# volser/FluidFramework

Measured on AMD Instinct MI355X. Metric: sequenced merge-tree ops applied/sec (whole node) + achieved HBM GB/s, higher is better.
Workload: dtype int32; 1 GPU; config2: 4096 docs x 8 clients x 10k msgs, lag U[0,32], 60/40 ins/rem; docs_per_gpu=4096, msgs_per_doc=10000, clients=8, lag_max=32, parallelism=doc-sharded x1, residency=blk, big_min_ops=0

## Files before the change

fluidframework_amd/csrc/mt_core.h:

```cpp
#pragma once
#include <type_traits>
#include "wave.h"
#include "../../include/mtgpu.h"

#define MT_MAXH 16
#define MT_PSK 16
#define MT_PKEYS MT_MAX_PROP_KEYS
#ifndef MT_PATH_RESUME
#define MT_PATH_RESUME 1
#endif
#define MT_MAXN 8
#define MT_GRAN 256
#define MT_ZMAX 2
#define MT_NOREM 0x7FFFFFFF
#define MT_RFL 128
#ifndef MT_L_ROWS
#define MT_L_ROWS 256
#endif
#ifndef MT_L_BLKS
#define MT_L_BLKS 96
#endif
#ifndef MT_L_HEAP
#define MT_L_HEAP 96
#endif
#define MT_L_H 8
#ifndef MT_B_BLKS
#define MT_B_BLKS 104
#endif
#ifndef MT_B_SLACK
#define MT_B_SLACK 13
#endif
#define MT_B_BT 128
#ifndef MT_B_W
#define MT_B_W 64
#endif
#ifndef MT_B_HEAP
#define MT_B_HEAP 94
#endif
#ifndef MT_BW_BLKS
#define MT_BW_BLKS 248
#endif
#ifndef MT_BW_W
#define MT_BW_W 256
#endif
#ifndef MT_BW_HEAP
#define MT_BW_HEAP 254
#endif
#define MT_BW_BT 256
#ifndef MT_G_U
#define MT_G_U 768
#endif
#ifndef MT_G_HEAP
#define MT_G_HEAP 2046
#endif
#ifndef MT_G_WIN
#define MT_G_WIN 2048
#endif
#define MT_G_H 12
#ifndef MT_G_BCACHE
#define MT_G_BCACHE 0
#endif
#ifndef MT_G_BC
#define MT_G_BC (MT_G_BCACHE ? 512 : 1)
#endif
#ifndef MT_G_BCH
#define MT_G_BCH 1
#endif
#define MT_BC_EMPTY ((int)0x80000000)
#ifndef MT_G_NW
#define MT_G_NW 4
#endif
#define MT_G_STG 1024
#ifndef MT_G_MWMIN
#define MT_G_MWMIN 512
#endif
#ifndef MT_G_ALLCH
#define MT_G_ALLCH 0
#endif
enum { MT_MW_EXIT = 0, MT_MW_SCAN = 1, MT_MW_CHAIN = 2, MT_MW_PREFETCH = 3 };
enum { MT_BIGF_NO_BCACHE = 1, MT_BIGF_NO_PREFETCH = 2, MT_BIGF_NO_TABLE = 4, MT_BIGF_NO_BPC = 8 };
#ifndef MT_G_HT
#define MT_G_HT 4096
#endif
#ifndef MT_G_BPC
#define MT_G_BPC 1
#endif
#define MT_G_BPL 11
#define MT_G_BP (1 << MT_G_BPL)
#define MT_BP_EMPTY 0xFFFFFFFFu
#define MT_G_HTN (MT_G_HT * 3 / 4)
enum { MT_RES_HBM = 0, MT_RES_LDS = 1, MT_RES_BLK = 2, MT_RES_BIG = 3, MT_RES_BLKW = 4 };
#if defined(MT_PROFILE) || defined(MT_PROFILE2) || defined(MT_PROFILE3) || defined(MT_PROFILE4) || defined(MT_BPC_STATS) || defined(MT_EVCOUNT3) || defined(MT_EVCOUNT) || defined(MT_EVCOUNT2)
#define MT_KEEP_PROF 1
#else
#define MT_KEEP_PROF 0
#endif

#if defined(MT_PROFILE) && defined(__HIP_DEVICE_COMPILE__)
#define MT_PB(v) const unsigned long long v = __builtin_amdgcn_s_memtime()
#define MT_PE(i, v) prof[i] += __builtin_amdgcn_s_memtime() - (v)
#else
#define MT_PB(v)
#define MT_PE(i, v)
#endif
#if defined(MT_EVCOUNT)
#define MT_EV(i, v) prof[i] += (unsigned long long)(v)
#else
#define MT_EV(i, v)
#endif
#if defined(MT_EVCOUNT2)
#define MT_EV2(i, v) prof[i] += (unsigned long long)(v)
#else
#define MT_EV2(i, v)
#endif
#if defined(MT_PROFILE2) && defined(__HIP_DEVICE_COMPILE__)
#define MT_QB(v) const unsigned long long v = __builtin_amdgcn_s_memtime()
#define MT_QE(i, v) prof[i] += __builtin_amdgcn_s_memtime() - (v)
#define MT_QC(i) prof[i] += 1
#else
#define MT_QB(v)
#define MT_QE(i, v)
#define MT_QC(i)
#endif
#if defined(MT_PROFILE3) && defined(__HIP_DEVICE_COMPILE__)
#define MT_ZB(v) const unsigned long long v = __builtin_amdgcn_s_memtime()
#define MT_ZE(i, v) prof[i] += __builtin_amdgcn_s_memtime() - (v)
#define MT_ZC(i) prof[i] += 1
#else
#define MT_ZB(v)
#define MT_ZE(i, v)
#define MT_ZC(i)
#endif
#if defined(MT_BPC_STATS) && !defined(__HIP_DEVICE_COMPILE__)
#define MT_BS(i) prof[i] += 1
#else
#define MT_BS(i)
#endif
#if defined(MT_PROFILE4) && defined(__HIP_DEVICE_COMPILE__)
#define MT_UB(v) const unsigned long long v = __builtin_amdgcn_s_memtime()
#define MT_UE(i, v) prof[i] += __builtin_amdgcn_s_memtime() - (v)
#define MT_UC(i, x) prof[i] += (unsigned long long)(x)
#else
#define MT_UB(v)
#define MT_UE(i, v)
#define MT_UC(i, x)
#endif
enum { MT_PH_U = 0, MT_PH_SPLIT, MT_PH_INSERT, MT_PH_RANGE, MT_PH_ZAMBONI, MT_PH_OP, MT_PH_GEN, MT_PH_TEXT };

#define MT_M_CLIENT 0x0000FFFFu
#define MT_M_REMOVED 0x00010000u
#define MT_M_MARKER 0x00020000u
#define MT_M_INWIN 0x00040000u
#define MT_M_REG 0x00080000u
#define MT_M_NONL 0x00100000u
#define MT_M_HREF1 0x01000000u
#define MT_M_HREF 0xFF000000u

#ifndef MT_ROW64
#define MT_ROW64 0
#endif
struct __attribute__((aligned(16))) MtRow {
    int len;
    int seq;
    int rseq;
    uint32_t meta;
    int toff;
    int props;
    int parent;
    int tcap;
    unsigned long long ovl;
    uint32_t rcl;
    int mid;
#if MT_ROW64
    int pad[4];
#endif
};
struct __attribute__((aligned(16))) MtBlk {
    int c[8];
    int len;
    int parent;
    int n;
    int height;
    int scour;
    int pad[3];
};
struct __attribute__((aligned(16))) MtPSet {
    uint16_t key[MT_PSK];
    int32_t val[MT_PSK];
    int32_t n;
    int32_t pad[3];
};
struct MtHeapE { int seg; int maxSeq; };
struct MtOvx { int row; int rseq; int client; int pad; };
#define MT_OVX_CAP 512
#define MT_REG_CAP 64
struct MtReg { int client, name, n, flags, off, pad[3]; };
// ... 69 lines not shown
    int32_t seq, rseq;
    uint16_t rclient; int16_t prop;
    uint32_t poff, plen;
    uint32_t mid, pad1;
};
enum { MT_LD_START = 0, MT_LD_CONT = 1, MT_LD_REFLUSH = 2, MT_LD_REFLUSH_NEW = 3, MT_LD_UNSUPPORTED = 4 };
struct MtLoadStep { int seg, kind, cli, seq; };
struct MtLoad {
    const uint32_t* docs; const uint32_t* seg_off; const uint32_t* nhdr;
    const int32_t* ms; const int32_t* cs;
    const MtLoadSeg* segs; const uint16_t* payload;
    const uint32_t* plan_off; const MtLoadStep* plan;
};
#define MT_NONCOLLAB 0xFFFE
#define MT_NOBODY 0xFFFF

struct MtGen {
    unsigned long long seed;
    uint32_t ops, clients, lag_max, pct_insert, pct_remove, ins_len_max, rem_len_max, n_ann_sets, pct_rewrite;
    int enabled;
    const uint32_t* clients_per_run;
    uint32_t doc_id_base;
    uint32_t ins_len_min, seg_prop_sets, ins_at_end;
    uint64_t total_ops;
};

struct __attribute__((aligned(16))) MtQ16 { uint32_t x, y, z, w; };
struct __attribute__((aligned(16))) MtLdsPools {
    MtRow rows[MT_L_ROWS];
    MtBlk blk[MT_L_BLKS];
    MtHeapE heap[MT_L_HEAP + 2];
    int win[MT_L_ROWS];
    int uid[MT_L_ROWS];
    int udelta[MT_L_ROWS];
    uint8_t uanc[MT_L_ROWS * MT_L_H];
};

template <int NB, int NH, int NT, int NW> struct __attribute__((aligned(16))) MtLdsBlkT {
    static_assert(NB <= NT, "block ids index the corrections table");
    MtBlk blk[NB];
    MtHeapE heap[NH + 2];
    int win[NW];
    int bcorr[NT];
};
using MtLdsBlk = MtLdsBlkT<MT_B_BLKS, MT_B_HEAP, MT_B_BT, MT_B_W>;
using MtLdsBlkW = MtLdsBlkT<MT_BW_BLKS, MT_BW_HEAP, MT_BW_BT, MT_BW_W>;

struct __attribute__((aligned(16))) MtLdsBig {
    MtHeapE heap[MT_G_HEAP + 2];
    int win[MT_G_WIN];
    int uid[MT_G_U], udelta[MT_G_U];
    int uanc[MT_G_U * MT_G_H];
    uint16_t ulist[MT_G_U];
    MtBlk bc[MT_G_BC];
    int btag[MT_G_BC];
    int sid[MT_G_STG], sdel[MT_G_STG], spf[MT_G_STG];
    int htk[MT_G_HT], htv[MT_G_HT];
    uint16_t hlist[MT_G_HT];
    uint32_t bpc[MT_G_BP];
    struct Job {
        int op, r, c, r0, n, H, minSeq, heapN;
        MtRow* R; int* win; MtBlk* blk; int* uanc; uint16_t* text;
    } mw[2];
    int posted;
};

struct MtScratch {
    int pathB[MT_MAXH + 2], pathJ[MT_MAXH + 2];
    int pathOff[MT_MAXH + 2], pathLen[MT_MAXH + 2];
    int hold[64];
    int holdLen[64];
    uint8_t holdBlk[64];
    int rfree[MT_RFL];
    int corr[MT_MAXN];
};

struct __attribute__((aligned(16), may_alias)) MtQ16a { uint32_t x, y, z, w; };
#ifndef MT_NONL
#define MT_NONL 1
#endif
#ifndef MT_LEAF_ONCE
#define MT_LEAF_ONCE 1
#endif
#ifndef MT_GT_CH
#define MT_GT_CH 4
#endif
#ifndef MT_SCOUR_QUADS
#define MT_SCOUR_QUADS 1
#endif
MT_INLINE int pick16(const int* c, int j) {
    int v = c[0];
#pragma unroll
    for (int i = 1; i < 16; i++) v = (j == i) ? c[i] : v;
    return v;
}
MT_INLINE int pick8(const int* c, int j) {
    int v = c[0];
#pragma unroll
    for (int i = 1; i < 8; i++) v = (j == i) ? c[i] : v;
    return v;
}
MT_INLINE bool ovl_has(const MtOvx* ox, int n, unsigned long long ovl, int s, int rseq, int c) {
    if (c < 63) return ((ovl >> c) & 1ull) != 0;
    const bool more = (ovl >> 63) != 0;
    bool f = false;
    for (int i = 0; i < n; i++) {
        const MtOvx e = ox[i];
        f = f | (more & (e.row == s) & (e.client == c) & (e.rseq == rseq));
    }
    return f;
}
MT_INLINE bool vis_rc(int seq, uint32_t meta, int rseq, uint32_t rcl, unsigned long long ovl, int r, int c,
                      const MtOvx* ox, int nox, int s) {
    const int cl = (int)(meta & MT_M_CLIENT);
    const bool seen = (cl == c) | (seq <= r);
    const bool removed = (meta & MT_M_REMOVED) != 0;
    const bool gone = ((int)rcl == c) | (rseq <= r) | ovl_has(ox, nox, ovl, s, rseq, c);
    return seen & !(removed & gone);
}

struct BlkH { int len, parent, n, height, scour; };
struct ChildL { int len; bool tie; };
struct WinI { int id; int delta; int parent; bool live; bool recycle; };

enum { MT_WALK_SPLIT = 0, MT_WALK_INSERT = 1 };
enum { MT_W_OK = 0, MT_W_NOCHANGE = 1, MT_W_FAIL = 2 };
enum { MT_MAP_REMOVE = 0, MT_MAP_ANNOTATE = 1, MT_MAP_COLLECT = 2 };
enum { MT_PM_SET = 0, MT_PM_REWRITE = 1, MT_PM_INCR = 2, MT_PM_KEEP = 3, MT_PM_CONS = 4, MT_PM_INCR_SMIN = 5 };
MT_INLINE int mt_prop_mode(uint32_t fl) {
    if (!(fl & MT_OPF_COMBINE)) return (fl & MT_OPF_REWRITE) ? MT_PM_REWRITE : MT_PM_SET;
    if (fl & MT_OPF_REWRITE) return (fl & MT_OPF_CONSENSUS) ? MT_PM_CONS : MT_PM_KEEP;
    return (fl & MT_OPF_INCR_STRMIN) ? MT_PM_INCR_SMIN : MT_PM_INCR;
}

struct MtEngParams {
    uint32_t rowCap, heapCap, winCap, textCap, psetCap, p_nsets;
    uint16_t* textBase;
    const uint32_t* p_off; const uint16_t* p_key; const int32_t* p_val;
    const uint8_t* p_falsy; const uint32_t* p_class; const int32_t* p_vinfo;
};
#if defined(__HIP_DEVICE_COMPILE__)
__shared__ MtLdsPools mt_lds_pools_v;
#else
static MtLdsPools mt_lds_pools_v;
#endif
MT_INLINE MtLdsPools& mt_lds() { return mt_lds_pools_v; }
#if defined(__HIP_DEVICE_COMPILE__)
__shared__ MtLdsBlk mt_ldsb_v;
#else
static MtLdsBlk mt_ldsb_v;
#endif
MT_INLINE MtLdsBlk& mt_ldsb() { return mt_ldsb_v; }
#if defined(__HIP_DEVICE_COMPILE__)
__shared__ MtLdsBlkW mt_ldsbw_v;
#else
static MtLdsBlkW mt_ldsbw_v;
#endif
MT_INLINE MtLdsBlkW& mt_ldsbw() { return mt_ldsbw_v; }
#if defined(__HIP_DEVICE_COMPILE__)
__shared__ MtLdsBig mt_ldsg_v;
#else
static MtLdsBig mt_ldsg_v;
#endif
MT_INLINE MtLdsBig& mt_ldsg() { return mt_ldsg_v; }

struct MtCold {
    MtEngParams S;
    uint32_t cnt[6];
    int hw[2];
    int lcap[3];
    uint32_t gcap[4];
    int epoch, ncol, midcap;
    uint32_t op;
    MtDocHdr* hdr; int* rfhbm; MtOvx* ovx; int* midt; MtReg* regs;
    MtBlk* blk; MtHeapE* heap; int *uid, *udelta, *uanc; MtPSet* pset;
    int ovxn, blkfreen, texthalf, psettop;
    uint16_t* dtext; unsigned long long dtcap;
    uint32_t dused, tused; int dstop;
    int* regr; int regTop, regHalf, regCap;
    int pcKey[4], pcVal[4];
    int pNever;
};
#if defined(__HIP_DEVICE_COMPILE__)
__shared__ MtCold mt_cold_v;
#else
static MtCold mt_cold_v;
#endif
#if defined(MT_DBG_FAIL) && defined(__HIP_DEVICE_COMPILE__)
struct MtDbg { int s, n; uint32_t op; };
__shared__ MtDbg mt_dbg_v;
#endif

template <int RES, bool FULL = true> struct MtEngT {
    static constexpr bool kFull = FULL;
    static constexpr bool LDS = RES == MT_RES_LDS;
    static constexpr bool BIG = RES == MT_RES_BIG;
    static constexpr bool BW = RES == MT_RES_BLKW;
    static constexpr bool BLKR = RES == MT_RES_BLK || BW;
    static constexpr bool BLKL = RES == MT_RES_LDS || BLKR;
    MT_HD auto& LB() const { if constexpr (BW) return mt_ldsbw(); else return mt_ldsb(); }
    MtEngParams& S = mt_cold_v.S;
    MtDocHdr*& hdrp = mt_cold_v.hdr;
    MtRow* R;
    template <class T> using Home = std::conditional_t<BLKR, T&, T>;
    int* win;
    Home<int*> uid = mt_cold_v.uid; Home<int*> udelta = mt_cold_v.udelta; Home<int*> uanc = mt_cold_v.uanc;
    Home<MtBlk*> blk = mt_cold_v.blk; Home<MtHeapE*> heap = mt_cold_v.heap;
    uint16_t* text; Home<MtPSet*> pset = mt_cold_v.pset;
    MtOvx*& ovx = mt_cold_v.ovx; int& ovxN = mt_cold_v.ovxn;
// ... 1315 lines not shown
    MT_HD void insertAtPath(int L, int idx, int node, int delta) {
        bool first = true;
        for (;;) {
            const int B = uni(sc->pathB[L]);
            BlkH h;
            auto cur = blkLoad(B, h);
            auto prv = wave_from8<-1>(cur);
            const int nd = node, ix = idx;
            auto nc = wave_map(8, [=](int i) MT_LAM {
                const int a = own(cur, i), b = own(prv, i);
                const int lt = -(int)(i < ix), eq = -(int)(i == ix);
                return (a & lt) | (nd & eq) | (b & ~(lt | eq));
            });
            const int n1 = h.n + 1;
            setChildParent(h.height, node, B);
            if (first) landB = B;
            if (n1 < MT_MAXN) {
                wave_for(8, [&](int i) MT_LAM { bk(B).c[i] = i < n1 ? own(nc, i) : -1; });
                bk(B).n = n1; bk(B).len = h.len + delta;
                if (delta != 0) wave_for(L, [&](int l) MT_LAM { const int pb = sc->pathB[l]; bk(pb).len = bk(pb).len + delta; });
                return;
            }
            lastSplit = true;
            MT_EV(6, 1);
            const int NB = allocBlock();
            if (NB < 0) return;
            auto hi = wave_from8<4>(nc);
            wave_for(8, [&](int i) MT_LAM {
                bk(NB).c[i] = i < 4 ? own(hi, i) : -1;
                bk(B).c[i] = i < 4 ? own(nc, i) : -1;
            });
            bk(NB).n = 4; bk(NB).height = h.height; bk(NB).scour = -1; bk(NB).parent = h.parent;
            bpPut(NB, h.parent);
            bk(B).n = 4;
            wave_for(4, [&](int i) MT_LAM { setChildParent(h.height, own(hi, i), NB); });
            if (first && ix >= 4) landB = NB;
            first = false;
            wave_sync();
            const int nbLen = sumObs(NB, 4, h.height), bLen = sumObs(B, 4, h.height);
            bk(NB).len = nbLen; bk(B).len = bLen;
            if (L == 0) {
                const int R = allocBlock();
                if (R < 0) return;
                wave_for(8, [&](int i) MT_LAM { bk(R).c[i] = i == 0 ? B : (i == 1 ? NB : -1); });
                bk(R).n = 2; bk(R).height = h.height + 1; bk(R).parent = -1; bk(R).scour = -1; bk(R).len = bLen + nbLen;
                bk(B).parent = R; bk(NB).parent = R;
                bpPut(R, -1); bpPut(B, R); bpPut(NB, R);
                root = R; height = h.height + 1;
                return;
            }
            node = NB; idx = uni(sc->pathJ[L - 1]) + 1; L = L - 1;
        }
    }
#if defined(MT_DBG_FAIL) && defined(__HIP_DEVICE_COMPILE__)
    __device__ void dbgWalkFail(int kind, int B, const BlkH& h, int ch, const ChildL& cl, int pos, int p, int total, int L,
                                int r, int c) {
        __builtin_amdgcn_s_waitcnt(0);
        __builtin_amdgcn_fence(__ATOMIC_SEQ_CST, "agent");
        const int lane = wave_lane();
        if (lane == 0)
            printf("WALKFAIL op=%u kind=%d B=%d height=%d n=%d hlen=%d L=%d root=%d H=%d pos=%d p=%d total=%d r=%d c=%d "
                   "minSeq=%d curSeq=%d uValid=%d nU=%d lastSplit(s=%d n=%d op=%u)\n",
                   curOp, kind, B, h.height, h.n, h.len, L, root, height, pos, p, total, r, c, minSeq, curSeq, (int)uValid, nU,
                   mt_dbg_v.s, mt_dbg_v.n, mt_dbg_v.op);
        if (lane < h.n) {
            if (h.height == 0) {
                const volatile MtRow* v = (const volatile MtRow*)&row(ch);
                const int ln = v->len, sq = v->seq, rs = v->rseq, par = v->parent;
                const uint32_t mt = v->meta, rc = v->rcl;
                const unsigned long long ov = v->ovl;
                const bool vis = vis_rc(sq, mt, rs, rc, ov, r, c, ovx, ovxN, ch);
                printf("  WALKFAIL child %d row=%d used_len=%d tie=%d | fresh len=%d seq=%d rseq=%d meta=%x rcl=%u ovl=%llx "
                       "parent=%d vis=%d\n", lane, ch, cl.len, (int)cl.tie, ln, sq, rs, mt, rc, ov, par, (int)vis);
            } else {
                int corr = 0;
                if constexpr (BT) corr = LB().bcorr[ch];
                const volatile MtBlk* v = (const volatile MtBlk*)&bk(ch);
                printf("  WALKFAIL child %d blk=%d used_len=%d | bk.len=%d bcorr=%d n=%d parent=%d height=%d\n", lane, ch, cl.len,
                       v->len, corr, v->n, v->parent, v->height);
            }
        }
    }
#endif
    MT_HD int walk(int kind, int pos, int r, int c, int cand, int candLen, int L0 = 0) {
        if (!(uValid && uRef == r && uCli == c)) { computeU(r, c, false); L0 = 0; }
        int B = root, L = 0, p = pos;
        if (L0 > 0) { B = uni(sc->pathB[L0]); L = L0; p = pos - uni(sc->pathOff[L0]); }
        const bool narrow = BIG && nU <= UCAP && !htOk;
        int lsN = -1;
        BlkH h;
        MT_QB(q0); MT_QC(2);
        auto ch = blkLoad(B, h);
        MT_QE(0, q0);
        for (;;) {
            MT_EV(5, 1);
            sc->pathB[L] = B;
            MT_QB(q1);
            const bool kpre = !BLKL && h.height > 0;
            LaneArr<int> r0{}, r1{};
            if (kpre) kidsLoad(ch, h.n, r0, r1);
            LaneArr<MtRow> lf{};
            LaneArr<ChildL> cl;
            if (MT_LEAF_ONCE && h.height == 0) {
                const int rr = r, cc = c;
                lf = wave_map(h.n, [&](int j) MT_LAM { return row(own(ch, j)); });
                cl = wave_map(h.n, [&](int j) MT_LAM {
                    const MtRow f = own(lf, j);
                    ChildL o;
                    o.len = vis_rc(f.seq, f.meta, f.rseq, f.rcl, f.ovl, rr, cc, ovx, ovxN, own(ch, j)) ? f.len : 0;
                    o.tie = !((f.meta & MT_M_REMOVED) && f.rseq <= rr);
                    return o;
                });
            } else cl = kpre ? childLens(B, h, ch, r, c, true, kidsLen(r0, r1), lsN) : childLens(B, h, ch, r, c);
            MT_QE(1, q1);
            auto lens = wave_map(h.n, [&](int j) MT_LAM { return own(cl, j).len; });
            auto pre = wave_excl_scan8(lens);
            const int total = wave_sum8(lens);
            sc->pathOff[L] = pos - p; sc->pathLen[L] = total;
            const bool interior = h.height > 0;
            auto cond = wave_map(h.n, [&](int j) MT_LAM {
                const int pj = p - own(pre, j), lj = own(cl, j).len;
                if (interior) return pj <= lj;
                return pj < lj || (pj == lj && pj == 0 && own(cl, j).tie);
            });
            const int j = wave_first(cond);
            if (j >= 0) {
                const int pj = p - wave_at(pre, j);
                if (interior) {
                    sc->pathJ[L] = j; L++; B = wave_at(ch, j); p = pj;
                    if (narrow && h.height > 1) lsN = narrowU(lsN, h.height - 1, B);
                    if (kpre) ch = kidRec(r0, r1, j, h, B); else ch = blkLoad(B, h);
                    continue;
                }
                const int s = wave_at(ch, j);
                lastL = L; lastSplit = false;
                if (kind == MT_WALK_SPLIT) {
                    const uint32_t sm = MT_LEAF_ONCE ? (uint32_t)wave_at(leafField(lf, j, 3), j) : uni(row(s).meta);
                    if (pj > 0 && !(sm & MT_M_MARKER)) {
                        const int n = MT_LEAF_ONCE ? splitRowKnown(s, pj, lf, j) : splitRow(s, pj);
                        if (n < 0) return MT_W_FAIL;
                        insertAtPath(L, j + 1, n, 0);
                        if (FULL && drec) {
                            const int ps = obsPosition(s);
                            const bool rm = (uni(row(s).meta) & MT_M_REMOVED) != 0;
                            emitDelta(MT_DK_SPLIT, ps, pj, s, n, uni(row(n).len));
                            (void)rm;
                        }
                        lastIdx = j + 1;
                        if (lastSplit) uValid = false;
                        return MT_W_OK;
                    }
                    lastIdx = j;
                    return MT_W_NOCHANGE;
                }
                insertAtPath(L, j, cand, candLen);
                uValid = false;
                return MT_W_OK;
            }
            if (p - total == 0) {
                lastL = L; lastIdx = h.n; lastSplit = false;
                if (kind == MT_WALK_SPLIT) return MT_W_NOCHANGE;
                insertAtPath(L, h.n, cand, candLen);
                uValid = false;
                return MT_W_OK;
            }
#if defined(MT_DBG_FAIL) && defined(__HIP_DEVICE_COMPILE__)
            dbgWalkFail(kind, B, h, ch, cl, pos, p, total, L, r, c);
#endif
            return MT_W_FAIL;
        }
    }

    MT_HD void heapAdd(int s, int ms) {
        if (heapN + 1 > (int)S.heapCap) { status |= MT_DS_OOM_HEAP; return; }
        int k = ++heapN;
        if (heapN > heapHW) heapHW = heapN;
        if (heapN < MT_WAVE) {
            const int n = heapN, dn = 31 - __builtin_clz((unsigned)n);
            auto mv = wave_map(n + 1, [&](int c) MT_LAM {
                c = mt_opaque(c);
                const int dc = 31 - __builtin_clz((unsigned)(c | 1));
                return (bool)((int)(c >= 2) & (int)((n >> (dn - dc)) == c));
            });
            auto pms = wave_map(n + 1, [&](int c) MT_LAM { return own(mv, c) ? (int)hp(mt_opaque(c) >> 1).maxSeq : 0; });
            auto psg = wave_map(n + 1, [&](int c) MT_LAM { return own(mv, c) ? (int)hp(mt_opaque(c) >> 1).seg : 0; });
            mv = wave_map(n + 1, [&](int c) MT_LAM { return own(mv, c) && own(pms, c) > ms; });
            const int top = wave_first(mv);
            k = top < 0 ? n : top >> 1;
            wave_for(n + 1, [&](int c) MT_LAM {
                if (own(mv, c)) { hp(c).seg = own(psg, c); hp(c).maxSeq = own(pms, c); }
                if (c == k) { hp(c).seg = s; hp(c).maxSeq = ms; }
            });
            if (k == 1) heapTop = ms;
            return;
        }
        while (k > 1) {
            const int pm = uni(hp(k >> 1).maxSeq);
            if (pm > ms) { hp(k).seg = hp(k >> 1).seg; hp(k).maxSeq = pm; k >>= 1; } else break;
        }
        hp(k).seg = s; hp(k).maxSeq = ms;
        if (k == 1) heapTop = ms;
    }
    MT_HD MtHeapE heapGet() {
        MT_EV(3, 1); MT_EV(7, heapN - 1);
        if (heapN < MT_WAVE) {
            const int N = heapN, n = N - 1;
            MtHeapE x; x.seg = uni(hp(1).seg); x.maxSeq = uni(hp(1).maxSeq);
            const int lseg = uni(hp(N).seg), lms = uni(hp(N).maxSeq);
            heapN = n;
            heapTop = 0x7FFFFFFF;
            if (n >= 1) {
                auto lm = wave_map(n + 1, [&](int i) MT_LAM { return (int)(i >= 1) & (int)(2 * i <= n) ? (int)hp(2 * mt_opaque(i)).maxSeq : 0; });
                auto rm = wave_map(n + 1, [&](int i) MT_LAM { return (int)(i >= 1) & (int)(2 * i < n) ? (int)hp(2 * mt_opaque(i) + 1).maxSeq : 0; });
                auto ls = wave_map(n + 1, [&](int i) MT_LAM { return (int)(i >= 1) & (int)(2 * i <= n) ? (int)hp(2 * mt_opaque(i)).seg : 0; });
                auto rs = wave_map(n + 1, [&](int i) MT_LAM { return (int)(i >= 1) & (int)(2 * i < n) ? (int)hp(2 * mt_opaque(i) + 1).seg : 0; });
                auto right = wave_map(n + 1, [&](int i) MT_LAM { return (bool)((int)(2 * i < n) & (int)(own(lm, i) > own(rm, i))); });
                auto cm = wave_map(n + 1, [&](int i) MT_LAM { return own(right, i) ? own(rm, i) : own(lm, i); });
                auto cs = wave_map(n + 1, [&](int i) MT_LAM { return own(right, i) ? own(rs, i) : own(ls, i); });
                auto nx = wave_map(n + 1, [&](int i) MT_LAM {
                    return (int)(i >= 1) & (int)(2 * i <= n) & (int)(own(cm, i) < lms) ? 2 * i + (int)own(right, i) : 0;
                });
                int k = 1;
                for (int t = wave_at(nx, 1); t != 0; t = wave_at(nx, t)) { MT_EV(4, 1); k = t; }
                const int dk = 31 - __builtin_clz((unsigned)k);
                wave_for(n + 1, [&](int i) MT_LAM {
                    if (i < 1 || i > k) return;
                    const int di = 31 - __builtin_clz((unsigned)i);
                    if ((k >> (dk - di)) != i) return;
                    if (i == k) { hp(i).seg = lseg; hp(i).maxSeq = lms; }
                    else { hp(i).seg = own(cs, i); hp(i).maxSeq = own(cm, i); }
                });
                heapTop = k == 1 ? lms : wave_at(cm, 1);
            }
            return x;
        }
        MtHeapE x; x.seg = uni(hp(1).seg); x.maxSeq = uni(hp(1).maxSeq);
        const int lseg = uni(hp(heapN).seg), lms = uni(hp(heapN).maxSeq);
        heapN--;
        heapTop = 0x7FFFFFFF;
        if (heapN >= 1) {
            int k = 1;
            heapTop = lms;
            while ((k << 1) <= heapN) {
                int j = k << 1;
                int hs = uni(hp(j).seg), hm = uni(hp(j).maxSeq);
                if (j < heapN) {
                    const int hm1 = uni(hp(j + 1).maxSeq);
                    if (hm > hm1) { j++; hs = uni(hp(j).seg); hm = hm1; }
                }
                if (lms <= hm) break;
                MT_EV(4, 1);
                if (k == 1) heapTop = hm;
                hp(k).seg = hs; hp(k).maxSeq = hm; k = j;
            }
            hp(k).seg = lseg; hp(k).maxSeq = lms;
        }
        return x;
    }
    MT_HD void addToLRUSet(int s, int sq) {
        if (!(sq > curSeq)) return;
        const int p = uni(row(s).parent);
        const uint32_t m = uni(row(s).meta);
        if (uni(bk(p).scour) != 1 && sq > curSeq) {
            bk(p).scour = 1;
            if ((m & MT_M_HREF) != MT_M_HREF) row(s).meta = m + MT_M_HREF1;
            heapAdd(s, sq);
        }
    }
    MT_HD void addToLRUSetKnown(int s, int sq, int p, uint32_t m) {
        if (!(sq > curSeq)) return;
        if (uni(bk(p).scour) != 1) {
            bk(p).scour = 1;
            if ((m & MT_M_HREF) != MT_M_HREF) row(s).meta = m + MT_M_HREF1;
            heapAdd(s, sq);
        }
    }
    MT_HD int pkey(int id, int i) const { return (int)pset[id + (i >> 4)].key[i & 15]; }
    MT_HD int pval(int id, int i) const { return pset[id + (i >> 4)].val[i & 15]; }
    MT_HD uint32_t pclass(int v) const { return v >= 0 ? S.p_class[v] : 0xFFFFFFFFu; }
    MT_HD bool pNeverMap(int a) const { return mt_cold_v.pNever && a >= 0 && uni(pset[a].pad[2]) != 0; }
    MT_HD bool propsMatch(int a, int b) {
        if (a == b) return !pNeverMap(a);
        if (a < 0 || b < 0) return false;
        const int na = uni(pset[a].n), nb = uni(pset[b].n);
        if (na != nb) return false;
        if constexpr (FULL) {
            if (__builtin_expect(na > MT_WAVE, 0)) return propsMatchWide(a, b, na);
        } else if (na > MT_WAVE) { status |= MT_DS_PROPS_TOO_MANY; return false; }
        auto ok = wave_map(na, [&](int k) MT_LAM {
            const int key = pkey(a, k);
            const uint32_t ca = pclass(pval(a, k));
            bool f = false;
            for (int i = 0; i < nb; i++) f |= (int)(pkey(b, i) == key) & (int)(pclass(pval(b, i)) == ca);
            return (f & (int)(ca != 0xFFFFFFFFu)) != 0;
        });
        return wave_count(ok) == na;
    }
    MT_HD bool propsMatchWide(int a, int b, int n) {
        for (int base = 0; base < n; base += MT_WAVE) {
            const int cnt = (n - base) < MT_WAVE ? (n - base) : MT_WAVE;
            auto ok = wave_map(cnt, [&](int k) MT_LAM {
                const int key = pkey(a, base + k);
                const uint32_t ca = pclass(pval(a, base + k));
                bool f = false;
                for (int i = 0; i < n; i++) f |= (int)(pkey(b, i) == key) & (int)(pclass(pval(b, i)) == ca);
                return (f & (int)(ca != 0xFFFFFFFFu)) != 0;
            });
            if (wave_count(ok) != cnt) return false;
        }
        return true;
// ... 576 lines not shown
            LaneArr<uint32_t> lm{}; LaneArr<int> lp{}, lr{};
            auto cl = h.height == 0 ? leafLens(ch, h.n, r, c, lm, lp, lr) : childLens(B, h, ch, r, c);
            auto lens = wave_map(h.n, [&](int j) MT_LAM { return own(cl, j).len; });
            const int j0 = wave_at(fJ, L);
            auto lensFrom = wave_map(h.n, [&](int j) MT_LAM { return j >= j0 ? own(lens, j) : 0; });
            auto pre = wave_excl_scan8(lensFrom);
            const int st = wave_at(fS, L), en = wave_at(fE, L);
            auto cond = wave_map(h.n, [&](int j) MT_LAM {
                const int lj = own(lens, j), pj = own(pre, j);
                return j >= j0 && (en - pj) > 0 && lj > 0 && (st - pj) < lj;
            });
            if (h.height == 0) {
                MT_EV2(7, 1);
                const int first = wave_first(cond);
                int obsDelta = 0;
                if (first >= 0) {
                    const int nact = wave_count(cond);
                    c_rows += 2ull * (uint64_t)nact;
                    if (mode == MT_MAP_COLLECT) {
                        const auto rk = wave_rank(cond);
                        const int k0 = regTop + nCol;
                        wave_for(h.n, [&](int j) MT_LAM {
                            if ((int)own(cond, j) & (int)(k0 + own(rk, j) < regCap)) regRow(k0 + own(rk, j)) = own(ch, j);
                        });
                        nCol += nact;
                    } else if (mode == MT_MAP_REMOVE) {
                        auto nd = wave_map(h.n, [&](int j) MT_LAM {
                            if (!own(cond, j)) return 0;
                            const int s = own(ch, j);
                            const uint32_t mt = own(lm, j);
                            if (mt & MT_M_REMOVED) {
                                row(s).ovl = row(s).ovl | (1ull << (c < 63 ? c : 63));
                                return 0;
                            }
                            row(s).meta = mt | MT_M_REMOVED;
                            row(s).rcl = (uint32_t)c;
                            row(s).rseq = sq;
                            return own(lr, j);
                        });
                        obsDelta = -wave_sum8(nd);
                        wave_sync();
                        if (c >= 63) {
                            const uint64_t ob = wave_ballot(wave_map(h.n, [&](int j) MT_LAM {
                                return (bool)((int)own(cond, j) & (int)(row(own(ch, j)).rseq != sq));
                            }));
                            for (uint64_t b = ob; b; b &= b - 1) {
                                const int j = __builtin_ctzll(b), s = wave_at(ch, j);
                                ovxAdd(s, uni(row(s).rseq), c);
                            }
                        }
                        winAddLanes(ch, cond, h.n);
                        if (rec) {
                            const int base = wave_at(fO, L);
                            auto ol = wave_map(h.n, [&](int j) MT_LAM {
                                const int g = own(ch, j); return (row(g).meta & MT_M_REMOVED) ? 0 : row(g).len;
                            });
                            auto opre = wave_excl_scan8(ol);
                            for (uint64_t b = wave_ballot(wave_map(h.n, [&](int j) MT_LAM { return own(nd, j) > 0; })); b; b &= b - 1) {
                                const int j = __builtin_ctzll(b);
                                emitDelta(MT_DK_REMOVE, base + wave_at(opre, j), wave_at(nd, j), wave_at(ch, j), -1, -1);
                            }
                        }
                    } else {
                        LaneArr<int> opre{};
                        int base = 0;
                        if (rec) {
                            base = wave_at(fO, L);
                            auto ol = wave_map(h.n, [&](int j) MT_LAM {
                                const int g = own(ch, j); return (row(g).meta & MT_M_REMOVED) ? 0 : row(g).len;
                            });
                            opre = wave_excl_scan8(ol);
                        }
                        for (int j = 0; j < h.n; j++) {
                            if (!wave_at(cond, j)) continue;
                            const int s = wave_at(ch, j);
                            const int old = wave_at(lp, j);
                            int nw;
                            if (old == lastOld) nw = lastNew;
                            else { nw = applyPropSet(old, opset, pm, sq); lastOld = old; lastNew = nw; }
                            row(s).props = nw;
                            if (rec) emitDelta(MT_DK_ANNOTATE, base + wave_at(opre, j), uni(row(s).len), s, old, nw);
                        }
                    }
                    if (mode != MT_MAP_COLLECT) addToLRUSet(wave_at(ch, first), sq);
                }
                if (mode == MT_MAP_REMOVE) bk(B).len = h.len + obsDelta;
                const int d = wave_at(fD, L) + obsDelta;
                L--;
                if (L < 0) topD = d;
                if (L >= 0) {
                    const int fl = wave_at(fL, L);
                    fD = wave_set(fD, L, wave_at(fD, L) + d); fS = wave_set(fS, L, wave_at(fS, L) - fl);
                    fE = wave_set(fE, L, wave_at(fE, L) - fl); fJ = wave_set(fJ, L, wave_at(fJ, L) + 1);
                }
                continue;
            }
            const int jj = wave_first(cond);
            if (jj >= 0) {
                const int pj = wave_at(pre, jj);
                fS = wave_set(fS, L, st - pj); fE = wave_set(fE, L, en - pj); fJ = wave_set(fJ, L, jj);
                fL = wave_set(fL, L, wave_at(lens, jj));
                int ob = 0;
                if (rec) ob = wave_at(fO, L) + wave_sum8(wave_map(h.n, [&](int i) MT_LAM { return i < jj ? bk(own(ch, i)).len : 0; }));
                const int child = wave_at(ch, jj);
                L++;
                fB = wave_set(fB, L, child); fJ = wave_set(fJ, L, 0); fS = wave_set(fS, L, st - pj);
                fE = wave_set(fE, L, en - pj); fD = wave_set(fD, L, 0); fO = wave_set(fO, L, ob);
                continue;
            }
            const int d = wave_at(fD, L);
            if (d != 0) bk(B).len = h.len + d;
            L--;
            if (L < 0) topD = d;
            if (L >= 0) {
                const int fl = wave_at(fL, L);
                fD = wave_set(fD, L, wave_at(fD, L) + d); fS = wave_set(fS, L, wave_at(fS, L) - fl);
                fE = wave_set(fE, L, wave_at(fE, L) - fl); fJ = wave_set(fJ, L, wave_at(fJ, L) + 1);
            }
        }
        if (L0 > 0 && topD != 0) {
            const int dd = topD;
            wave_for(L0, [&](int l) MT_LAM { const int pb = sc->pathB[l]; bk(pb).len = bk(pb).len + dd; });
            wave_sync();
        }
        uValid = false;
    }
    MT_HD void loadHeader(const MtLoad& Ld, uint32_t s0, int nh, int ms, int cs) {
        minSeq = ms; curSeq = cs;
        if (nh == 0) return;
        if (nh > (int)S.rowCap) { status |= MT_DS_OOM_ROWS; return; }
        const MtLoadSeg* G = Ld.segs + s0;
        const uint32_t pbase = uni(G[0].poff);
        int ttot = 0;
        for (int base = 0; base < nh; base += MT_WAVE) {
            const int m = (nh - base) < MT_WAVE ? (nh - base) : MT_WAVE;
            auto tl = wave_map(m, [&](int k) MT_LAM {
                const MtLoadSeg g = G[base + k];
                return (g.flags & MT_LS_MARKER) ? 0 : (int)g.plen;
            });
            ttot += wave_sum(tl);
        }
        if (ttot > (int)S.textCap) { status |= MT_DS_OOM_TEXT; return; }
        const int t0 = textTop;
        for (int base = 0; base < nh; base += MT_WAVE) {
            const int m = (nh - base) < MT_WAVE ? (nh - base) : MT_WAVE;
            wave_for(m, [&](int k) MT_LAM {
                const MtLoadSeg g = G[base + k];
                const int s = base + k;
                const bool mk = (g.flags & MT_LS_MARKER) != 0, rm = (g.flags & MT_LS_REMOVED) != 0;
                const int cl = (g.flags & MT_LS_CLIENT) ? (int)g.client : MT_NONCOLLAB;
                MtRow& w = row(s);
                w.len = mk ? 1 : (int)g.plen;
                w.seq = (g.flags & MT_LS_SEQ) ? g.seq : 0;
                w.rseq = rm ? g.rseq : MT_NOREM;
                w.meta = (uint32_t)cl | (rm ? MT_M_REMOVED : 0u) | (mk ? MT_M_MARKER : 0u);
                w.rcl = rm ? (uint32_t)g.rclient : 0u;
                w.ovl = 0ull; w.props = -1; w.parent = -1;
                w.mid = mk ? (int)g.mid : 0;
                if (mk && g.mid && !rm && (int)g.mid <= midCap) midt[g.mid - 1] = s;
                w.toff = mk ? (int)g.plen : t0 + (int)(g.poff - pbase);
                w.tcap = mk ? 0 : (int)g.plen;
            });
        }
        for (int base = 0; base < ttot; base += MT_WAVE) {
            const int m = (ttot - base) < MT_WAVE ? (ttot - base) : MT_WAVE;
            wave_for(m, [&](int k) MT_LAM { text[t0 + base + k] = Ld.payload[pbase + base + k]; });
        }
// ... 188 lines not shown
                row(d).toff = row(s).toff; row(d).tcap = (mt & MT_M_MARKER) ? 0 : row(s).len;
                row(d).ovl = 0ull; row(d).parent = -1;
                regRow(base + i) = d;
                return (mt & MT_M_REMOVED) != 0;
            });
            rem |= wave_ballot(rm);
        }
        rfN = n < f0 ? f0 - n : 0;
        rowTop = t0 + (n > f0 ? n - f0 : 0);
        wave_sync();
        MtReg& g = regs[e];
        const int on = uni(g.client) == c ? uni(g.n) : 0, of = uni(g.flags), oo = uni(g.off);
        if (on > 0 && !(of & 2)) {
            for (int i = 0; i < on; i++) {
                const int s = uni(regRow(oo + i));
                row(s).meta = uni(row(s).meta) & ~MT_M_REG;
                freeRow(s);
            }
        }
        const int fl = rem ? 1 : 0;
        wave_for(1, [&](int) MT_LAM { g.client = c; g.name = name; g.n = n; g.flags = fl; g.off = base; });
        regTop = base + n;
        wave_sync();
    }
    MT_HD void regCompact() {
        const auto ns = wave_map(MT_REG_CAP, [&](int i) MT_LAM { return regs[i].client >= 0 ? regs[i].n : 0; });
        const auto os = wave_map(MT_REG_CAP, [&](int i) MT_LAM { return regs[i].off; });
        const int other = regHalf ^ 1;
        int* dst = regr + (size_t)other * regCap;
        int w = 0;
        for (int e = 0; e < MT_REG_CAP; e++) {
            const int n = wave_at(ns, e), o = wave_at(os, e);
            if (n <= 0) continue;
            for (int b0 = 0; b0 < n; b0 += MT_WAVE) {
                const int m = (n - b0) < MT_WAVE ? (n - b0) : MT_WAVE;
                wave_for(m, [&](int k) MT_LAM { dst[w + b0 + k] = regRow(o + b0 + k); });
            }
            const int w0 = w;
            wave_for(1, [&](int) MT_LAM { regs[e].off = w0; });
            w += n;
        }
        wave_sync();
        regHalf = other; regTop = w;
    }
    MT_HD void opPaste(int pos, int r, int c, int sq, int name) {
        const int e = regFind(c, name, false);
        if (e < 0) return;
        MtReg& g = regs[e];
        const int n = uni(g.n), fl = uni(g.flags), o = uni(g.off);
        if (n == 0) return;
        if (fl & 3) { status |= MT_DS_UNSUPPORTED; return; }
        if (walk(MT_WALK_SPLIT, pos, r, c, -1, 0) == MT_W_OK) c_rows += 2;
        if (status) return;
        int ip = pos;
        for (int i = 0; i < n; i++) {
            const int k = uni(regRow(o + i));
            const uint32_t mt = (uni(row(k).meta) & ~(MT_M_REG | MT_M_CLIENT)) | (uint32_t)c;
            const int L = uni(row(k).len);
            row(k).meta = mt; row(k).seq = sq;
            const int mi = uni(row(k).mid);
            if ((mt & MT_M_MARKER) && mi > 0 && mi <= midCap) midt[mi - 1] = k;
            wave_sync();
            landB = -1;
            const int w = walk(MT_WALK_INSERT, ip, r, c, k, L);
            if (w != MT_W_OK || landB < 0) { status |= MT_DS_INSERT_FAILED; return; }
            c_rows += 2;
            const uint32_t m1 = winAddKnown(k, mt);
            if (sq > minSeq) addToLRUSetKnown(k, sq, landB, m1);
            if (FULL && drec) {
                if (mt & MT_M_MARKER) emitDelta(MT_DK_INSERT, obsPosition(k), L, k, uni(row(k).props), 1, uni(row(k).toff));
                else {
                    const int to = dText(uni(row(k).toff), L);
                    emitDelta(MT_DK_INSERT, obsPosition(k), L, k, uni(row(k).props), 0, to);
                }
            }
            ip += L;
        }
        wave_for(1, [&](int) MT_LAM { g.flags = fl | 2; });
        wave_sync();
        zamboni();
    }
    MT_HD void opRange(int mode, int start, int end, int r, int c, int sq, int opset, int pm) {
        MT_PB(t0);
        int w = walk(MT_WALK_SPLIT, start, r, c, -1, 0);
        if (w == MT_W_OK) c_rows += 2;
        if (status) return;
        int L0 = 0;
        if (MT_PATH_RESUME && w != MT_W_FAIL && !lastSplit && uValid && uRef == r && uCli == c) {
            for (int l = lastL; l > 0; l--) {
                if (end - uni(sc->pathOff[l]) <= uni(sc->pathLen[l])) { L0 = l; break; }
            }
        }
        w = walk(MT_WALK_SPLIT, end, r, c, -1, 0, L0);
        if (w == MT_W_OK) c_rows += 2;
        if (status) return;
        if (w == MT_W_FAIL || lastSplit || !uValid) L0 = 0;
        MT_PE(MT_PH_SPLIT, t0);
        MT_PB(t1);
        rangeMap(mode, start, end, r, c, sq, opset, pm, L0);
        MT_PE(MT_PH_RANGE, t1);
        if (status) return;
        zamboni();
    }
};
using MtEng = MtEngT<MT_RES_HBM>;
using MtEngFast = MtEngT<MT_RES_HBM, false>;

template <class Eng>
MT_HD void mt_load_doc(Eng& e, const MtLoad& Ld, uint32_t i) {
    const uint32_t s0 = Ld.seg_off[i], p0 = Ld.plan_off[i], p1 = Ld.plan_off[i + 1];
    if (p1 > p0 && uni(Ld.plan[p0].kind) == MT_LD_UNSUPPORTED) { e.status |= MT_DS_UNSUPPORTED; return; }
    e.loadHeader(Ld, s0, (int)Ld.nhdr[i], Ld.ms[i], Ld.cs[i]);
    int pos = 0, prevLen = 0;
    for (uint32_t k = p0; k < p1 && !e.status; k++) {
        const MtLoadStep st = Ld.plan[k];
        const int kind = uni(st.kind);
        if (kind == MT_LD_REFLUSH || kind == MT_LD_REFLUSH_NEW) {
            const int p = uni(e.bk(e.root).len);
            if (p <= e.perspectiveLength(0, MT_NONCOLLAB)) e.status |= MT_DS_UNSUPPORTED;
            else if (kind == MT_LD_REFLUSH_NEW) e.status |= MT_DS_INSERT_FAILED;
            continue;
        }
        if (kind == MT_LD_UNSUPPORTED) { e.status |= MT_DS_UNSUPPORTED; break; }
        pos = kind == MT_LD_START ? uni(e.bk(e.root).len) : pos + prevLen;
        prevLen = e.loadInsert(Ld, s0 + (uint32_t)uni(st.seg), pos, uni(st.cli), uni(st.seq), kind == MT_LD_START);
        if (!e.status) e.zamboni();
    }
}
```

Before: 271.5 million ops/s.

## Apply range ops within a single leaf in one fused walk pass

Adds a fast path to the split walk so that when a remove or annotate range starts and ends inside the same leaf block, both boundary splits, the removal or annotation marks, window registration and ancestor length updates happen in one wave-parallel pass. This avoids the second walk for the end position and the separate rangeMap traversal. It falls back to the old path when there is no room for two splits, capacity is short, overlap bits are set, or delta recording is on. The general rangeMap also now passes known metadata to the LRU update instead of re-reading the row. The fast path adds a lot of intricate row-rewriting code, which raises correctness risk and register pressure.

```diff
diff --git a/fluidframework_amd/csrc/mt_core.h b/fluidframework_amd/csrc/mt_core.h
--- a/fluidframework_amd/csrc/mt_core.h
+++ b/fluidframework_amd/csrc/mt_core.h
@@ -90,7 +90,7 @@
 #define MT_BP_EMPTY 0xFFFFFFFFu
 #define MT_G_HTN (MT_G_HT * 3 / 4)
 enum { MT_RES_HBM = 0, MT_RES_LDS = 1, MT_RES_BLK = 2, MT_RES_BIG = 3, MT_RES_BLKW = 4 };
-#if defined(MT_PROFILE) || defined(MT_PROFILE2) || defined(MT_PROFILE3) || defined(MT_PROFILE4) || defined(MT_BPC_STATS) || defined(MT_EVCOUNT3) || defined(MT_EVCOUNT) || defined(MT_EVCOUNT2)
+#if defined(MT_PROFILE) || defined(MT_PROFILE2) || defined(MT_PROFILE3) || defined(MT_PROFILE4) || defined(MT_BPC_STATS) || defined(MT_EVCOUNT3) || defined(MT_EVCOUNT) || defined(MT_EVCOUNT2) || defined(MT_EVRANGE)
 #define MT_KEEP_PROF 1
 #else
 #define MT_KEEP_PROF 0
@@ -112,6 +112,11 @@
 #define MT_EV2(i, v) prof[i] += (unsigned long long)(v)
 #else
 #define MT_EV2(i, v)
+#endif
+#if defined(MT_EVRANGE)
+#define MT_EVR(i, v) prof[i] += (unsigned long long)(v)
+#else
+#define MT_EVR(i, v)
 #endif
 #if defined(MT_PROFILE2) && defined(__HIP_DEVICE_COMPILE__)
 #define MT_QB(v) const unsigned long long v = __builtin_amdgcn_s_memtime()
@@ -347,6 +352,9 @@
 #ifndef MT_LEAF_ONCE
 #define MT_LEAF_ONCE 1
 #endif
+#ifndef MT_RANGE_LEAF
+#define MT_RANGE_LEAF 1
+#endif
 #ifndef MT_GT_CH
 #define MT_GT_CH 4
 #endif
@@ -388,8 +396,8 @@
 struct ChildL { int len; bool tie; };
 struct WinI { int id; int delta; int parent; bool live; bool recycle; };
 
-enum { MT_WALK_SPLIT = 0, MT_WALK_INSERT = 1 };
-enum { MT_W_OK = 0, MT_W_NOCHANGE = 1, MT_W_FAIL = 2 };
+enum { MT_WALK_SPLIT = 0, MT_WALK_INSERT = 1, MT_WALK_RANGE = 2 };
+enum { MT_W_OK = 0, MT_W_NOCHANGE = 1, MT_W_FAIL = 2, MT_W_RANGED = 3 };
 enum { MT_MAP_REMOVE = 0, MT_MAP_ANNOTATE = 1, MT_MAP_COLLECT = 2 };
 enum { MT_PM_SET = 0, MT_PM_REWRITE = 1, MT_PM_INCR = 2, MT_PM_KEEP = 3, MT_PM_CONS = 4, MT_PM_INCR_SMIN = 5 };
 MT_INLINE int mt_prop_mode(uint32_t fl) {
@@ -1871,7 +1879,128 @@
         }
     }
 #endif
-    MT_HD int walk(int kind, int pos, int r, int c, int cand, int candLen, int L0 = 0) {
+    MT_HD bool rangeLeaf(int B, int L, const BlkH& h, const LaneArr<int>& ch, const LaneArr<MtRow>& lf,
+                         const LaneArr<ChildL>& cl, const LaneArr<int>& pre, int total, int p, int j, int span, int mode,
+                         int c, int sq, int opset, int pm) {
+        const int n = h.n, pe = p + span;
+        if (span <= 0 || pe > total) return false;
+        MT_EVR(2, 1);
+        if (c >= 63 || mode > MT_MAP_ANNOTATE || (FULL && drec != nullptr)) { MT_EVR(4, 1); return false; }
+        const auto len = wave_map(n, [&](int i) MT_LAM { return own(cl, i).len; });
+        const auto meta = wave_map(n, [&](int i) MT_LAM { return own(lf, i).meta; });
+        const auto ce = wave_map(n, [&](int i) MT_LAM {
+            const int q = pe - own(pre, i), l = own(len, i);
+            return (bool)((int)(q < l) | ((int)(q == 0) & (int)(l == 0) & (int)own(cl, i).tie));
+        });
+        const int je = wave_first(ce);
+        const int pj = p - wave_at(pre, j), pje = je >= 0 ? pe - wave_at(pre, je) : 0;
+        const uint32_t mj = wave_at(meta, j), mje = je >= 0 ? wave_at(meta, je) : 0u;
+        const int s1 = (int)(pj > 0) & (int)!(mj & MT_M_MARKER), s2 = (int)(pje > 0) & (int)!(mje & MT_M_MARKER);
+        const int ns = s1 + s2;
+        if (n + ns >= MT_MAXN) { MT_EVR(3, 1); return false; }
+        const auto cov = wave_map(n, [&](int i) MT_LAM {
+            const int q = own(pre, i), l = own(len, i);
+            return (bool)((int)(l > 0) & (int)(pe - q > 0) & (int)(p - q < l));
+        });
+        const bool rem = mode == MT_MAP_REMOVE;
+        const auto add = wave_map(n, [&](int i) MT_LAM {
+            return (bool)((int)own(cov, i) & (int)!(own(meta, i) & MT_M_INWIN) & (int)rem);
+        });
+        const bool side = wave_ballot(wave_map(n, [&](int i) MT_LAM {
+            return (bool)((int)own(cov, i) & (int)(own(lf, i).ovl >> 63));
+        })) != 0;
+        const int w1 = s1 & (int)((mj & MT_M_INWIN) != 0), w2 = s2 & (int)((mje & MT_M_INWIN) != 0);
+        const int nadd = wave_count(add);
+        if (side || rfN + ((int)S.rowCap - rowTop) < ns || winN + w1 + w2 + nadd > (int)S.winCap) {
+            MT_EVR(4, 1);
+            return false;
+        }
+        MT_EVR(1, 1); MT_EVR(5, ns); MT_EV2(5, ns); MT_EV2(7, 1);
+        int n1 = -1, n2 = -1;
+        if (s1) n1 = allocRow();
+        if (s2) n2 = allocRow();
+        const int nact = wave_count(cov), first = wave_first(cov);
+        const unsigned long long cbit = 1ull << c;
+        const auto nd = wave_map(n, [&](int i) MT_LAM {
+            const MtRow f = own(lf, i);
+            const int isS = (int)(i == j) & s1, isE = (int)(i == je) & s2, isC = (int)own(cov, i);
+            if (isE) {
+                MtQ16a* d = (MtQ16a*)&row(n2);
+                d[0] = MtQ16a{(uint32_t)(f.len - pje), (uint32_t)f.seq, (uint32_t)f.rseq, f.meta & ~MT_M_HREF};
+                d[1] = MtQ16a{(uint32_t)(f.toff + pje), (uint32_t)f.props, (uint32_t)B, (uint32_t)(f.tcap - pje)};
+                d[2] = MtQ16a{(uint32_t)f.ovl, (uint32_t)(f.ovl >> 32), f.rcl, 0u};
+            }
+            const int lo = isS ? pj : 0, hi = isE ? pje : f.len;
+            if (isS) {
+                ((MtQ16a*)&row(n1))[1] =
+                    MtQ16a{(uint32_t)(f.toff + pj), (uint32_t)f.props, (uint32_t)B, (uint32_t)((isE ? pje : f.tcap) - pj)};
+            }
+            if (isS | isE) row(own(ch, i)).tcap = isS ? pj : pje;
+            const int gone = (int)((f.meta & MT_M_REMOVED) != 0);
+            const int mark = isC & (int)rem, fresh = mark & (gone ^ 1);
+            const uint32_t crs = fresh ? (uint32_t)sq : (uint32_t)f.rseq, crc = fresh ? (uint32_t)c : f.rcl;
+            const unsigned long long cov_ovl = (mark & gone) ? f.ovl | cbit : f.ovl;
+            const uint32_t cm = mark ? f.meta | MT_M_REMOVED | MT_M_INWIN : f.meta;
+            const int here = isC & (isS ^ 1);
+            MtQ16a* own_ = (MtQ16a*)&row(own(ch, i));
+            if (isS | isE | (here & mark))
+                own_[0] = MtQ16a{(uint32_t)(isS ? pj : hi), (uint32_t)f.seq, here ? crs : (uint32_t)f.rseq, here ? cm : f.meta};
+            if (here & mark) own_[2] = MtQ16a{(uint32_t)cov_ovl, (uint32_t)(cov_ovl >> 32), crc, (uint32_t)f.mid};
+            if (isS) {
+                MtQ16a* d = (MtQ16a*)&row(n1);
+                d[0] = MtQ16a{(uint32_t)(hi - pj), (uint32_t)f.seq, crs, cm & ~MT_M_HREF};
+                d[2] = MtQ16a{(uint32_t)cov_ovl, (uint32_t)(cov_ovl >> 32), crc, 0u};
+            }
+            return fresh ? hi - lo : 0;
+        });
+        const int obsDelta = -wave_sum8(nd);
+        if (mode == MT_MAP_ANNOTATE) {
+            const auto old = wave_map(n, [&](int i) MT_LAM { return own(lf, i).props; });
+            const auto pid = wave_map(n, [&](int i) MT_LAM { return ((int)(i == j) & s1) ? n1 : own(ch, i); });
+            int lastOld = -2, lastNew = -1;
+            for (uint64_t b = wave_ballot(cov); b; b &= b - 1) {
+                const int i = __builtin_ctzll(b), o = wave_at(old, i);
+                if (o != lastOld) { lastNew = applyPropSet(o, opset, pm, sq); lastOld = o; }
+                row(wave_at(pid, i)).props = lastNew;
+            }
+        }
+        if (w1) winSet(winN++, n1);
+        if (w2) winSet(winN++, n2);
+        if (nadd) {
+            const auto rk = wave_rank(add);
+            const int w0 = winN;
+            wave_for(n, [&](int i) MT_LAM {
+                if (own(add, i)) winSet(w0 + own(rk, i), ((int)(i == j) & s1) ? n1 : own(ch, i));
+            });
+            winN += nadd;
+        }
+        if (winN > winHW) winHW = winN;
+        if (ns) {
+            wave_for(n, [&](int i) MT_LAM { bk(B).c[i + (s1 & (int)(i > j)) + (s2 & (int)(i > je))] = own(ch, i); });
+            if (s1) bk(B).c[j + 1] = n1;
+            if (s2) bk(B).c[je + 1 + s1] = n2;
+            bk(B).n = n + ns;
+            landB = B;
+        }
+        if (rem) {
+            bk(B).len = h.len + obsDelta;
+            if (L > 0 && obsDelta != 0) {
+                wave_for(L, [&](int l) MT_LAM { const int pb = sc->pathB[l]; bk(pb).len = bk(pb).len + obsDelta; });
+                wave_sync();
+            }
+        }
+        if (first >= 0) {
+            const bool half = first == j && s1;
+            const uint32_t m0 = half ? mj & ~MT_M_HREF : wave_at(meta, first);
+            addToLRUSetKnown(half ? n1 : wave_at(ch, first), sq, B, rem ? m0 | MT_M_REMOVED | MT_M_INWIN : m0);
+        }
+        c_rows += 2u * (uint32_t)(ns + nact);
+        lastL = L; lastSplit = false; uValid = false;
+        lastIdx = je < 0 ? n + s1 : (s2 ? je + 1 + s1 : je + (s1 & (int)(je > j)));
+        return true;
+    }
+    MT_HD int walk(int kind, int pos, int r, int c, int cand, int candLen, int L0 = 0, int rEnd = 0, int rMode = 0,
+                   int rSq = 0, int rOpset = -1, int rPm = 0) {
         if (!(uValid && uRef == r && uCli == c)) { computeU(r, c, false); L0 = 0; }
         int B = root, L = 0, p = pos;
         if (L0 > 0) { B = uni(sc->pathB[L0]); L = L0; p = pos - uni(sc->pathOff[L0]); }
@@ -1923,7 +2052,11 @@
                 }
                 const int s = wave_at(ch, j);
                 lastL = L; lastSplit = false;
-                if (kind == MT_WALK_SPLIT) {
+                if (MT_RANGE_LEAF && MT_LEAF_ONCE && kind == MT_WALK_RANGE) {
+                    if (rangeLeaf(B, L, h, ch, lf, cl, pre, total, p, j, rEnd - pos, rMode, c, rSq, rOpset, rPm))
+                        return MT_W_RANGED;
+                }
+                if (kind != MT_WALK_INSERT) {
                     const uint32_t sm = MT_LEAF_ONCE ? (uint32_t)wave_at(leafField(lf, j, 3), j) : uni(row(s).meta);
                     if (pj > 0 && !(sm & MT_M_MARKER)) {
                         const int n = MT_LEAF_ONCE ? splitRowKnown(s, pj, lf, j) : splitRow(s, pj);
@@ -1948,7 +2081,7 @@
             }
             if (p - total == 0) {
                 lastL = L; lastIdx = h.n; lastSplit = false;
-                if (kind == MT_WALK_SPLIT) return MT_W_NOCHANGE;
+                if (kind != MT_WALK_INSERT) return MT_W_NOCHANGE;
                 insertAtPath(L, h.n, cand, candLen);
                 uValid = false;
                 return MT_W_OK;
@@ -2014,7 +2147,7 @@
                 const int dk = 31 - __builtin_clz((unsigned)k);
                 wave_for(n + 1, [&](int i) MT_LAM {
                     if (i < 1 || i > k) return;
-                    const int di = 31 - __builtin_clz((unsigned)i);
+                    const int di = 31 - __builtin_clz((unsigned)mt_opaque(i));
                     if ((k >> (dk - di)) != i) return;
                     if (i == k) { hp(i).seg = lseg; hp(i).maxSeq = lms; }
                     else { hp(i).seg = own(cs, i); hp(i).maxSeq = own(cm, i); }
@@ -2757,7 +2890,12 @@
                             if (rec) emitDelta(MT_DK_ANNOTATE, base + wave_at(opre, j), uni(row(s).len), s, old, nw);
                         }
                     }
-                    if (mode != MT_MAP_COLLECT) addToLRUSet(wave_at(ch, first), sq);
+                    if (mode != MT_MAP_COLLECT) {
+                        if (MT_RANGE_LEAF && !status) {
+                            const uint32_t m0 = wave_at(lm, first);
+                            addToLRUSetKnown(wave_at(ch, first), sq, B, mode == MT_MAP_REMOVE ? m0 | MT_M_REMOVED | MT_M_INWIN : m0);
+                        } else addToLRUSet(wave_at(ch, first), sq);
+                    }
                 }
                 if (mode == MT_MAP_REMOVE) bk(B).len = h.len + obsDelta;
                 const int d = wave_at(fD, L) + obsDelta;
@@ -3112,7 +3250,14 @@
     }
     MT_HD void opRange(int mode, int start, int end, int r, int c, int sq, int opset, int pm) {
         MT_PB(t0);
-        int w = walk(MT_WALK_SPLIT, start, r, c, -1, 0);
+        MT_EVR(0, 1);
+        int w = walk(MT_RANGE_LEAF ? MT_WALK_RANGE : MT_WALK_SPLIT, start, r, c, -1, 0, 0, end, mode, sq, opset, pm);
+        if (MT_RANGE_LEAF && w == MT_W_RANGED) {
+            MT_PE(MT_PH_SPLIT, t0);
+            if (status) return;
+            zamboni();
+            return;
+        }
         if (w == MT_W_OK) c_rows += 2;
         if (status) return;
         int L0 = 0;
```

New measurement: 276.6 million ops/s, median of 6. 1.9% higher.
